# AIGeeksGroup/UniVid

Measured on AMD Instinct MI355X. Metric: denoise_steps_per_sec, higher is better.
Workload: dtype bf16

## Files before the change

### univid_amd/csrc/gemm_bf16_kernels.h

```cpp
#pragma once
#include "common.h"
#include <stdlib.h>
#include <type_traits>

const float* uv_zero_page();

#define UV_BK 64

enum {
    UV_EPI_BF16 = 0,
    UV_EPI_GELU_BF16 = 1,
    UV_EPI_F32_FROM_BF16 = 2,
    UV_EPI_RESID_F32 = 3,
    UV_EPI_GATE_RESID_F32 = 4,
    UV_EPI_BF16_T = 5,
    UV_EPI_BF16_SSQ = 6,
};

struct GemmArgs {
    const bf16_t* A;
    const bf16_t* W;
    const bf16_t* bias;
    void* out;
    const float* gate;
    const int32_t* gate_tid;
    const float* zeros;
    long lda, ldw, ldo, gate_stride;
    int M, N, K;
    int tiles_m, tiles_n;
    int gm;
    float* ssq;
    long ld_ssq;
    float* ws_slab;
    int* ws_cnt;
};

typedef __attribute__((address_space(3))) void lds_void;

__device__ __forceinline__ void glds16(const void* g, lds_void* l) {
    __builtin_amdgcn_global_load_lds(g, l, 16, 0, 0);
}

template <int EPI, bool F16 = false, bool FULL = false>
__device__ __forceinline__ void epi_frag(const GemmArgs& p, int mb, int nb, const f32x4& a, int frow, int fq) {
    if (EPI != UV_EPI_BF16_T) {
        const int m = mb + frow, n = nb + 4 * fq;
        if (!FULL && (m >= p.M || n >= p.N)) return;
        float v[4];
#pragma unroll
        for (int e = 0; e < 4; ++e) v[e] = a[e];
        if (FULL || p.bias) {
            const u32x2 bb = *(const u32x2*)((FULL && !p.bias) ? (const bf16_t*)p.zeros : p.bias + n);
            v[0] += in16<F16>((bf16_t)(bb[0] & 0xffff));
            v[1] += in16<F16>((bf16_t)(bb[0] >> 16));
            v[2] += in16<F16>((bf16_t)(bb[1] & 0xffff));
            v[3] += in16<F16>((bf16_t)(bb[1] >> 16));
        }
        if (EPI == UV_EPI_BF16) {
            u32x2 o = {pack16_2<F16>(v[0], v[1]), pack16_2<F16>(v[2], v[3])};
            *(u32x2*)((bf16_t*)p.out + (long)m * p.ldo + n) = o;
        } else if (EPI == UV_EPI_GELU_BF16) {
#pragma unroll
            for (int e = 0; e < 4; e += 2) {
                const uint32_t pk = pack16_2<F16>(v[e], v[e + 1]);
                const f32x2 y = gelu_tanh_f32x2((f32x2){in16<F16>((bf16_t)(pk & 0xffff)), in16<F16>((bf16_t)(pk >> 16))});
                v[e] = y[0];
                v[e + 1] = y[1];
            }
            u32x2 o = {pack16_2<F16>(v[0], v[1]), pack16_2<F16>(v[2], v[3])};
            *(u32x2*)((bf16_t*)p.out + (long)m * p.ldo + n) = o;
        } else if (EPI == UV_EPI_F32_FROM_BF16) {
            f32x4 o = {round16<F16>(v[0]), round16<F16>(v[1]), round16<F16>(v[2]), round16<F16>(v[3])};
            *(f32x4*)((float*)p.out + (long)m * p.ldo + n) = o;
        } else if (EPI == UV_EPI_RESID_F32) {
            float* xp = (float*)p.out + (long)m * p.ldo + n;
            f32x4 x = *(const f32x4*)xp;
#pragma unroll
            for (int e = 0; e < 4; ++e) x[e] = __fadd_rn(x[e], round16<F16>(v[e]));
            *(f32x4*)xp = x;
        } else if (EPI == UV_EPI_GATE_RESID_F32) {
            const int t = p.gate_tid ? p.gate_tid[m] : 0;
            const f32x4 g = *(const f32x4*)(p.gate + (long)t * p.gate_stride + n);
            float* xp = (float*)p.out + (long)m * p.ldo + n;
            f32x4 x = *(const f32x4*)xp;
#pragma unroll
            for (int e = 0; e < 4; ++e) x[e] = __fadd_rn(x[e], __fmul_rn(round16<F16>(v[e]), g[e]));
            *(f32x4*)xp = x;
        }
    } else {
        const int n = nb + frow, m = mb + 4 * fq;
        if (!FULL && (n >= p.N || m >= p.M)) return;
        const float b = FULL ? in16<F16>(*(p.bias ? p.bias + n : (const bf16_t*)p.zeros)) : (p.bias ? in16<F16>(p.bias[n]) : 0.f);
        bf16_t* op = (bf16_t*)p.out + (long)n * p.ldo + m;
        if (FULL || m + 3 < p.M) {
            u32x2 o = {pack16_2<F16>(a[0] + b, a[1] + b), pack16_2<F16>(a[2] + b, a[3] + b)};
            *(u32x2*)op = o;
        } else {
            for (int e = 0; e < 4 && m + e < p.M; ++e) op[e] = out16<F16>(a[e] + b);
        }
    }
}


__device__ __forceinline__ float ssq_group32(const float (&v0)[4], const float (&v1)[4]) {
    const float s0 = __fadd_rn(__fadd_rn(__fadd_rn(__fmul_rn(v0[0], v0[0]), __fmul_rn(v0[1], v0[1])), __fmul_rn(v0[2], v0[2])), __fmul_rn(v0[3], v0[3]));
    const float s1 = __fadd_rn(__fadd_rn(__fadd_rn(__fmul_rn(v1[0], v1[0]), __fmul_rn(v1[1], v1[1])), __fmul_rn(v1[2], v1[2])), __fmul_rn(v1[3], v1[3]));
    const float u = __fadd_rn(s0, s1);
    const float t = __fadd_rn(u, __shfl_xor(u, 16, 64));
    return __fadd_rn(t, __shfl_xor(t, 32, 64));
}

template <bool F16>
__device__ __forceinline__ void epi_pair_ssq(const GemmArgs& p, int mb, int nb, const f32x4& a0, const f32x4& a1, int frow, int fq) {
    const int m = mb + frow;
    float v[2][4];
#pragma unroll
    for (int f = 0; f < 2; ++f) {
        const int n = min(nb + 16 * f + 4 * fq, p.N - 4);
        const u32x2 bb = p.bias ? *(const u32x2*)(p.bias + n) : (u32x2){0u, 0u};
        const f32x4& a = f ? a1 : a0;
        v[f][0] = round16<F16>(a[0] + in16<F16>((bf16_t)(bb[0] & 0xffff)));
        v[f][1] = round16<F16>(a[1] + in16<F16>((bf16_t)(bb[0] >> 16)));
        v[f][2] = round16<F16>(a[2] + in16<F16>((bf16_t)(bb[1] & 0xffff)));
        v[f][3] = round16<F16>(a[3] + in16<F16>((bf16_t)(bb[1] >> 16)));
        if (m < p.M && nb + 16 * f + 4 * fq < p.N) {
            u32x2 o = {pack16_2<F16>(v[f][0], v[f][1]), pack16_2<F16>(v[f][2], v[f][3])};
            *(u32x2*)((bf16_t*)p.out + (long)m * p.ldo + nb + 16 * f + 4 * fq) = o;
        }
    }
    const float g = ssq_group32(v[0], v[1]);
    if (fq == 0 && m < p.M && nb < p.N) p.ssq[(long)m * p.ld_ssq + (nb >> 5)] = g;
}

template <int EPI, bool F16>
__device__ __forceinline__ void epi_pair16(const GemmArgs& p, int mb, int nb, const f32x4& a0, const f32x4& a1, int frow, int fq) {
    static_assert(EPI == UV_EPI_BF16 || EPI == UV_EPI_GELU_BF16 || EPI == UV_EPI_BF16_SSQ, "16-bit row-major outputs only");
    const int m = mb + frow;
    uint32_t w[2][2];
    float r[2][4];
#pragma unroll
    for (int f = 0; f < 2; ++f) {
        const int n = nb + 16 * f + 4 * fq;
        const u32x2 bb = *(const u32x2*)(p.bias ? p.bias + n : (const bf16_t*)p.zeros);
        const f32x4& a = f ? a1 : a0;
        float v[4] = {a[0] + in16<F16>((bf16_t)(bb[0] & 0xffff)), a[1] + in16<F16>((bf16_t)(bb[0] >> 16)),
                      a[2] + in16<F16>((bf16_t)(bb[1] & 0xffff)), a[3] + in16<F16>((bf16_t)(bb[1] >> 16))};
        if (EPI == UV_EPI_GELU_BF16) {
#pragma unroll
            for (int e = 0; e < 4; e += 2) {
                const uint32_t pk = pack16_2<F16>(v[e], v[e + 1]);
                const f32x2 r = {in16<F16>((bf16_t)(pk & 0xffff)), in16<F16>((bf16_t)(pk >> 16))};
                const f32x2 y = gelu_tanh_f32x2(r);
                v[e] = y[0];
                v[e + 1] = y[1];
            }
        }
        if (EPI == UV_EPI_BF16_SSQ) {
#pragma unroll
            for (int e = 0; e < 4; ++e) r[f][e] = v[e] = round16<F16>(v[e]);
        }
        w[f][0] = pack16_2<F16>(v[0], v[1]);
        w[f][1] = pack16_2<F16>(v[2], v[3]);
    }
    if (EPI == UV_EPI_BF16_SSQ) {
        const float g = ssq_group32(r[0], r[1]);
        if (fq == 0) p.ssq[(long)m * p.ld_ssq + (nb >> 5)] = g;
    }
    const auto s0 = __builtin_amdgcn_permlane16_swap(w[0][0], w[1][0], false, false);
    const auto s1 = __builtin_amdgcn_permlane16_swap(w[0][1], w[1][1], false, false);
    const u32x4 o = {(uint32_t)s0[0], (uint32_t)s1[0], (uint32_t)s0[1], (uint32_t)s1[1]};
    const int col = ((fq & 1) << 4) + ((fq >> 1) << 3);
    *(u32x4*)((bf16_t*)p.out + (long)m * p.ldo + nb + col) = o;
}

template <bool F16>
__device__ __forceinline__ void epi_pair16_T(const GemmArgs& p, int mb, int nb, const f32x4& a0, const f32x4& a1, int frow, int fq) {
    const int n = nb + frow;
    const float b = in16<F16>(*(p.bias ? p.bias + n : (const bf16_t*)p.zeros));
    uint32_t w0[2] = {pack16_2<F16>(a0[0] + b, a0[1] + b), pack16_2<F16>(a0[2] + b, a0[3] + b)};
    uint32_t w1[2] = {pack16_2<F16>(a1[0] + b, a1[1] + b), pack16_2<F16>(a1[2] + b, a1[3] + b)};
    const auto s0 = __builtin_amdgcn_permlane16_swap(w0[0], w1[0], false, false);
    const auto s1 = __builtin_amdgcn_permlane16_swap(w0[1], w1[1], false, false);
    const u32x4 o = {(uint32_t)s0[0], (uint32_t)s1[0], (uint32_t)s0[1], (uint32_t)s1[1]};
    const int row = ((fq & 1) << 4) + ((fq >> 1) << 3);
    *(u32x4*)((bf16_t*)p.out + (long)n * p.ldo + mb + row) = o;
}

template <int EPI, int NF, int D, bool F16 = false>
__device__ __forceinline__ void epi_rmw_pipe(const GemmArgs& p, const int (&mb)[NF], const int (&nb)[NF], const f32x4 (&acc)[NF],
                                             int frow, int fq) {
    static_assert(EPI == UV_EPI_RESID_F32 || EPI == UV_EPI_GATE_RESID_F32, "rmw epilogues only");
    constexpr bool GATE = EPI == UV_EPI_GATE_RESID_F32;
    const float* grow[NF];
    if (GATE) {
        int t[NF];
#pragma unroll
        for (int f = 0; f < NF; ++f) t[f] = p.gate_tid ? p.gate_tid[min(mb[f] + frow, p.M - 1)] : 0;
#pragma unroll
        for (int f = 0; f < NF; ++f) grow[f] = p.gate + (long)t[f] * p.gate_stride;
    }
    f32x4 xb[D], gb[D];
    u32x2 bb[D];
    auto issue = [&](int f, int slot) {
        const int m = min(mb[f] + frow, p.M - 1), n = min(nb[f] + 4 * fq, p.N - 4);
        xb[slot] = *(const f32x4*)((const float*)p.out + (long)m * p.ldo + n);
        if (GATE) gb[slot] = *(const f32x4*)(grow[f] + n);
        bb[slot] = p.bias ? *(const u32x2*)(p.bias + n) : (u32x2){0u, 0u};
    };
#pragma unroll
    for (int f = 0; f < D && f < NF; ++f) issue(f, f);
#pragma unroll
    for (int f = 0; f < NF; ++f) {
        const int slot = f % D;
        const int m = mb[f] + frow, n = nb[f] + 4 * fq;
        float v[4];
        v[0] = acc[f][0] + in16<F16>((bf16_t)(bb[slot][0] & 0xffff));
        v[1] = acc[f][1] + in16<F16>((bf16_t)(bb[slot][0] >> 16));
        v[2] = acc[f][2] + in16<F16>((bf16_t)(bb[slot][1] & 0xffff));
        v[3] = acc[f][3] + in16<F16>((bf16_t)(bb[slot][1] >> 16));
        f32x4 x = xb[slot];
#pragma unroll
        for (int e = 0; e < 4; ++e)
            x[e] = GATE ? __fadd_rn(x[e], __fmul_rn(round16<F16>(v[e]), gb[slot][e])) : __fadd_rn(x[e], round16<F16>(v[e]));
        if (m < p.M && n < p.N) *(f32x4*)((float*)p.out + (long)m * p.ldo + n) = x;
        if (f + D < NF) issue(f + D, slot);
    }
}

template <int BM, int BN, int WM, int WN, int EPI, int NS = 2, bool F16 = false>
__global__ __launch_bounds__(WM* WN * 64) void gemm_bf16_nt_kernel(GemmArgs p) {
    constexpr int NW = WM * WN;
    constexpr int NT = NW * 64;
    constexpr int TM = BM / WM / 16;
    constexpr int TN = BN / WN / 16;
    constexpr int A_BYTES = BM * 128;
    constexpr int W_BYTES = BN * 128;
    constexpr int STAGE_BYTES = A_BYTES + W_BYTES;
    constexpr int A_INSTR = (BM / 8 + NW - 1) / NW;
    constexpr int W_INSTR = (BN / 8 + NW - 1) / NW;
    static_assert(BM % 8 == 0 && BN % 8 == 0 && (BM / WM) % 16 == 0 && (BN / WN) % 16 == 0, "tile/wave mismatch");
    constexpr bool TRANS = (EPI == UV_EPI_BF16_T);

    extern __shared__ __attribute__((aligned(16))) char smem[];

    const int tid = threadIdx.x;
    const int lane = tid & 63;
    const int wave = __builtin_amdgcn_readfirstlane(tid >> 6);
    const int wm = wave / WN, wn = wave % WN;

    const int nblk = p.tiles_m * p.tiles_n;
    int bid = blockIdx.x;
    {
        const int q = nblk >> 3, r = nblk & 7, xcd = bid & 7, idx = bid >> 3;
        bid = (xcd < r ? xcd * (q + 1) : r * (q + 1) + (xcd - r) * q) + idx;
    }
    constexpr int GM = 4;
    const int group_sz = GM * p.tiles_n;
    const int group = bid / group_sz;
    const int first_m = group * GM;
    const int gm = min(GM, p.tiles_m - first_m);
    const int in_group = bid - group * group_sz;
    const int tile_m = first_m + in_group % gm;
    const int tile_n = in_group / gm;
    const int m0 = tile_m * BM, n0 = tile_n * BN;

    const int srow = lane >> 3;
    const int pchunk = lane & 7;
    const bf16_t* a_src[A_INSTR];
    const bf16_t* w_src[W_INSTR];
#pragma unroll
    for (int i = 0; i < A_INSTR; ++i) {
        const int row = (i * NW + wave) * 8 + srow;
        const int c = pchunk ^ ((row >> 1) & 7);
        const int gr = min(m0 + row, p.M - 1);
        a_src[i] = p.A + (long)gr * p.lda + c * 8;
    }
#pragma unroll
    for (int i = 0; i < W_INSTR; ++i) {
        const int row = (i * NW + wave) * 8 + srow;
        const int c = pchunk ^ ((row >> 1) & 7);
        const int gr = min(n0 + row, p.N - 1);
        w_src[i] = p.W + (long)gr * p.ldw + c * 8;
    }

    auto stage = [&](int kt, int buf) {
        char* base = smem + buf * STAGE_BYTES;
        const int koff = kt * UV_BK;
#pragma unroll
        for (int i = 0; i < A_INSTR; ++i)
            if ((i * NW + wave) * 8 < BM) glds16(a_src[i] + koff, (lds_void*)(base + (i * NW + wave) * 1024));
#pragma unroll
        for (int i = 0; i < W_INSTR; ++i)
            if ((i * NW + wave) * 8 < BN) glds16(w_src[i] + koff, (lds_void*)(base + A_BYTES + (i * NW + wave) * 1024));
    };

    f32x4 acc[TN][TM];
#pragma unroll
    for (int i = 0; i < TN; ++i)
#pragma unroll
        for (int j = 0; j < TM; ++j) acc[i][j] = (f32x4){0.f, 0.f, 0.f, 0.f};

    const int frow = lane & 15;
    const int fq = lane >> 4;
    int a_off[TM], w_off[TN];
    int a_key[TM], w_key[TN];
#pragma unroll
    for (int j = 0; j < TM; ++j) {
        const int row = wm * (BM / WM) + j * 16 + frow;
        a_off[j] = row * 128;
        a_key[j] = (row >> 1) & 7;
    }
#pragma unroll
    for (int i = 0; i < TN; ++i) {
        const int row = wn * (BN / WN) + i * 16 + frow;
        w_off[i] = A_BYTES + row * 128;
        w_key[i] = (row >> 1) & 7;
    }

    const int nk = p.K / UV_BK;
    auto compute = [&](const char* base) {
#pragma unroll
        for (int ks = 0; ks < 2; ++ks) {
            bf16x8 af[TM], wf[TN];
            const int c = ks * 4 + fq;
#pragma unroll
            for (int j = 0; j < TM; ++j)
                af[j] = *(const bf16x8*)(base + a_off[j] + ((c ^ a_key[j]) << 4));
#pragma unroll
            for (int i = 0; i < TN; ++i)
                wf[i] = *(const bf16x8*)(base + w_off[i] + ((c ^ w_key[i]) << 4));
#pragma unroll
            for (int i = 0; i < TN; ++i)
#pragma unroll
                for (int j = 0; j < TM; ++j) {
                    if (TRANS)
                        acc[i][j] = mfma_16x16x32<F16>(af[j], wf[i], acc[i][j]);
                    else
                        acc[i][j] = mfma_16x16x32<F16>(wf[i], af[j], acc[i][j]);
                }
        }
    };
    if constexpr (NS == 2) {
        stage(0, 0);
        asm volatile("s_waitcnt vmcnt(0)" ::: "memory");
        __syncthreads();
        for (int kt = 0; kt < nk; ++kt) {
            const int buf = kt & 1;
            if (kt + 1 < nk) stage(kt + 1, buf ^ 1);
            compute(smem + buf * STAGE_BYTES);
            asm volatile("s_waitcnt vmcnt(0)" ::: "memory");
            __syncthreads();
        }
    } else {
        static_assert(BM % (8 * NW) == 0 && BN % (8 * NW) == 0, "ring variant needs unguarded staging");
        constexpr int LPS = A_INSTR + W_INSTR;
        static_assert((NS - 2) * LPS < 64, "vmcnt range");
#pragma unroll
        for (int s0 = 0; s0 < NS - 1; ++s0)
            if (s0 < nk) stage(s0, s0);
        int buf = 0, nbuf = NS - 1;
        for (int kt = 0; kt < nk; ++kt) {
            if (kt + NS - 2 < nk) {
                asm volatile("s_waitcnt vmcnt(%0)" ::"n"((NS - 2) * LPS) : "memory");
            } else {
                asm volatile("s_waitcnt vmcnt(0)" ::: "memory");
            }
            __builtin_amdgcn_s_barrier();
            if (kt + NS - 1 < nk) stage(kt + NS - 1, nbuf);
            compute(smem + buf * STAGE_BYTES);
            buf = buf + 1 == NS ? 0 : buf + 1;
            nbuf = nbuf + 1 == NS ? 0 : nbuf + 1;
        }
    }

    if constexpr (EPI == UV_EPI_RESID_F32 || EPI == UV_EPI_GATE_RESID_F32) {
        constexpr int NF = TM * TN;
        int mb[NF], nb[NF];
        f32x4 av[NF];
#pragma unroll
        for (int j = 0; j < TM; ++j)
#pragma unroll
            for (int i = 0; i < TN; ++i) {
                mb[j * TN + i] = m0 + wm * (BM / WM) + j * 16;
                nb[j * TN + i] = n0 + wn * (BN / WN) + i * 16;
                av[j * TN + i] = acc[i][j];
            }
        epi_rmw_pipe<EPI, NF, (NF >= 8 ? 4 : 2), F16>(p, mb, nb, av, frow, fq);
    } else if constexpr (EPI == UV_EPI_BF16_SSQ) {
        static_assert(TN % 2 == 0 && (BN / WN) % 32 == 0, "UV_EPI_BF16_SSQ needs whole 32-column groups per wave");
#pragma unroll
        for (int j = 0; j < TM; ++j)
#pragma unroll
            for (int i = 0; i < TN; i += 2)
                epi_pair_ssq<F16>(p, m0 + wm * (BM / WM) + j * 16, n0 + wn * (BN / WN) + i * 16, acc[i][j], acc[i + 1][j], frow, fq);
    } else {
#pragma unroll
        for (int j = 0; j < TM; ++j)
#pragma unroll
            for (int i = 0; i < TN; ++i)
                epi_frag<EPI, F16>(p, m0 + wm * (BM / WM) + j * 16, n0 + wn * (BN / WN) + i * 16, acc[i][j], frow, fq);
    }
}


template <int EPI, bool F16>
__device__ __forceinline__ void epi_rmw_rows_lds(const GemmArgs& p, char* smem, const f32x4 (&acc)[2][2][2][4], int m0, int n0,
                                                 int wave, int lane) {
    static_assert(EPI == UV_EPI_RESID_F32 || EPI == UV_EPI_GATE_RESID_F32, "rmw epilogues only");
    constexpr bool GATE = EPI == UV_EPI_GATE_RESID_F32;
    constexpr int D = 8;
    const int wr = wave >> 2, wc = wave & 3;
    const int frow = lane & 15, fq = lane >> 4;
    float bv[2][2][4];
#pragma unroll
    for (int hn = 0; hn < 2; ++hn)
#pragma unroll
        for (int i = 0; i < 2; ++i) {
            const int n = min(n0 + hn * 128 + wc * 32 + i * 16 + 4 * fq, p.N - 4);
            const u32x2 bb = p.bias ? *(const u32x2*)(p.bias + n) : (u32x2){0u, 0u};
            bv[hn][i][0] = in16<F16>((bf16_t)(bb[0] & 0xffff));
            bv[hn][i][1] = in16<F16>((bf16_t)(bb[0] >> 16));
            bv[hn][i][2] = in16<F16>((bf16_t)(bb[1] & 0xffff));
            bv[hn][i][3] = in16<F16>((bf16_t)(bb[1] >> 16));
        }
    const int n = n0 + 4 * lane;
    const bool n_ok = n < p.N;
    const int nc = min(n, p.N - 4);
#pragma unroll
    for (int h = 0; h < 2; ++h) {
#pragma unroll
        for (int j = 0; j < 4; ++j)
#pragma unroll
            for (int hn = 0; hn < 2; ++hn)
#pragma unroll
                for (int i = 0; i < 2; ++i) {
                    const int row = wr * 64 + j * 16 + frow;
                    const int chunk = hn * 32 + wc * 8 + i * 4 + fq;
                    f32x4 y;
#pragma unroll
                    for (int e = 0; e < 4; ++e) y[e] = round16<F16>(acc[hn][h][i][j][e] + bv[hn][i][e]);
                    *(f32x4*)(smem + row * 1024 + ((chunk ^ (row & 7)) << 4)) = y;
                }
        asm volatile("s_waitcnt lgkmcnt(0)" ::: "memory");
        __builtin_amdgcn_s_barrier();
        const int mbase = m0 + h * 128 + wave * 16;
        f32x4 xb[D], gb[D];
        int tid16 = 0;
        if (GATE && p.gate_tid) tid16 = p.gate_tid[min(mbase + (lane & 15), p.M - 1)];
        auto issue = [&](int rr, int slot) {
            const int m = min(mbase + rr, p.M - 1);
            xb[slot] = *(const f32x4*)((const float*)p.out + (long)m * p.ldo + nc);
            if (GATE) {
                const int t = __builtin_amdgcn_readlane(tid16, rr);
                gb[slot] = *(const f32x4*)(p.gate + (long)t * p.gate_stride + nc);
            }
        };
#pragma unroll
        for (int rr = 0; rr < D; ++rr) issue(rr, rr);
#pragma unroll
        for (int rr = 0; rr < 16; ++rr) {
            const int slot = rr % D;
            const int row = wave * 16 + rr;
            const f32x4 y = *(const f32x4*)(smem + row * 1024 + ((lane ^ (row & 7)) << 4));
            f32x4 x = xb[slot];
#pragma unroll
            for (int e = 0; e < 4; ++e) x[e] = GATE ? __fadd_rn(x[e], __fmul_rn(y[e], gb[slot][e])) : __fadd_rn(x[e], y[e]);
            if (mbase + rr < p.M && n_ok) *(f32x4*)((float*)p.out + (long)(mbase + rr) * p.ldo + n) = x;
            if (rr + D < 16) issue(rr + D, slot);
        }
        if (h == 0) {
            asm volatile("s_waitcnt lgkmcnt(0)" ::: "memory");
            __builtin_amdgcn_s_barrier();
        }
    }
}

#define UV_SB() __builtin_amdgcn_s_barrier()
#define UV_SCHED() __builtin_amdgcn_sched_barrier(0)

template <int EPI, int VAR = 0, bool F16 = false, int SK = 1>
__global__ __launch_bounds__(512) void gemm_bf16_8ph_kernel(GemmArgs p) {
    static_assert(SK == 1 || (VAR == 5 && (8 % SK) == 0), "split-K: VAR 5, SK in {2, 4, 8}");
    constexpr bool TRANS = (EPI == UV_EPI_BF16_T);
    constexpr int HALF = 16384;
    constexpr int BUF = 4 * HALF;
    extern __shared__ __attribute__((aligned(16))) char smem[];

    const int tid = threadIdx.x;
    const int lane = tid & 63;
    const int wave = __builtin_amdgcn_readfirstlane(tid >> 6);
    const int wr = wave >> 2, wc = wave & 3;

    const int nblk = p.tiles_m * p.tiles_n;
    int bid = blockIdx.x;
    int slice = 0;
    if constexpr (SK == 1) {
        const int q = nblk >> 3, r = nblk & 7, xcd = bid & 7, idx = bid >> 3;
        bid = (xcd < r ? xcd * (q + 1) : r * (q + 1) + (xcd - r) * q) + idx;
    } else {
        const int xcd = bid & 7, idx = bid >> 3, per = gridDim.x >> 3;
        const int u = xcd * per + idx;
        slice = u % SK;
        bid = u / SK;
        if (bid >= nblk) return;
    }
    constexpr int GM = 4;
    const int group_sz = GM * p.tiles_n;
    const int group = bid / group_sz;
    const int first_m = group * GM;
    const int gm = min(GM, p.tiles_m - first_m);
    const int in_group = bid - group * group_sz;
    const int m0 = (first_m + in_group % gm) * 256, n0 = (in_group / gm) * 256;
    const int kbeg = SK == 1 ? 0 : slice * (p.K / SK);

    const int srow = lane >> 3, pchunk = lane & 7;
    const bf16_t* a_src[2][2];
    const bf16_t* w_src[2][2];
#pragma unroll
    for (int h = 0; h < 2; ++h)
#pragma unroll
        for (int i = 0; i < 2; ++i) {
            const int row = (i * 8 + wave) * 8 + srow;
            const int c = pchunk ^ ((row >> 1) & 7);
            a_src[h][i] = p.A + (long)min(m0 + h * 128 + row, p.M - 1) * p.lda + c * 8 + kbeg;
            w_src[h][i] = p.W + (long)min(n0 + h * 128 + row, p.N - 1) * p.ldw + c * 8 + kbeg;
        }
    char* const my_dst = smem + wave * 1024;
    const int nk = p.K / SK / UV_BK;
#define UV_STAGE(SRC, KT, DSTOFF)                                         \
    {                                                                     \
        const bf16_t* g0_ = SRC[0] + (long)(KT) * UV_BK;                  \
        const bf16_t* g1_ = SRC[1] + (long)(KT) * UV_BK;                  \
        glds16(g0_, (lds_void*)(my_dst + (DSTOFF)));                      \
        glds16(g1_, (lds_void*)(my_dst + (DSTOFF) + 8192));              \
    }

    const int frow = lane & 15, fq = lane >> 4;
    const int lx = (fq ^ (frow >> 1)) << 4;
    const char* const la = smem + (wr * 64 + frow) * 128;
    const char* const lw = smem + 2 * HALF + (wc * 32 + frow) * 128;

    f32x4 acc[2][2][2][4];
#pragma unroll
    for (int a = 0; a < 2; ++a)
#pragma unroll
        for (int b = 0; b < 2; ++b)
#pragma unroll
            for (int i = 0; i < 2; ++i)
#pragma unroll
                for (int j = 0; j < 4; ++j) acc[a][b][i][j] = (f32x4){0.f, 0.f, 0.f, 0.f};
    bf16x8 af[4][2], w0[2][2], w1[2][2];

#define UV_RD_A(B, H)                                                                             \
    _Pragma("unroll") for (int j = 0; j < 4; ++j) {                                                                     \
        af[j][0] = *(const bf16x8*)(la + (B) * BUF + (H) * HALF + j * 2048 + lx);                 \
        af[j][1] = *(const bf16x8*)(la + (B) * BUF + (H) * HALF + j * 2048 + (lx ^ 64));          \
    }
#define UV_RD_W(B, H, WF)                                                                         \
    _Pragma("unroll") for (int i = 0; i < 2; ++i) {                                                                     \
        WF[i][0] = *(const bf16x8*)(lw + (B) * BUF + (H) * HALF + i * 2048 + lx);                 \
        WF[i][1] = *(const bf16x8*)(lw + (B) * BUF + (H) * HALF + i * 2048 + (lx ^ 64));          \
    }
#define UV_MFMA_H(HM, HN, WF, KS)                                                                 \
    _Pragma("unroll") for (int i = 0; i < 2; ++i)                                                 \
    _Pragma("unroll") for (int j = 0; j < 4; ++j) {                                               \
        if (TRANS)                                                                                \
            acc[HN][HM][i][j] = mfma_16x16x32<F16>(af[j][KS], WF[i][KS], acc[HN][HM][i][j]); \
        else                                                                                      \
            acc[HN][HM][i][j] = mfma_16x16x32<F16>(WF[i][KS], af[j][KS], acc[HN][HM][i][j]); \
    }
#define UV_MFMA_Q(HM, HN, WF)                                                                     \
    __builtin_amdgcn_s_setprio(1);                                                                \
    UV_MFMA_H(HM, HN, WF, 0) UV_MFMA_H(HM, HN, WF, 1)                                             \
    __builtin_amdgcn_s_setprio(0);
#define UV_LGKM0() asm volatile("s_waitcnt lgkmcnt(0)" ::: "memory")
#define UV_KTILE0(T, B, O, ST1, ST2)                                                              \
    UV_RD_W(B, 0, w0) UV_SCHED(); UV_RD_A(B, 0)                                                   \
    if (ST1) UV_STAGE(a_src[1], (T) + 1, (O) * BUF + HALF)                                        \
    asm volatile("s_waitcnt lgkmcnt(8)" ::: "memory");                                            \
    UV_SB(); UV_LGKM0(); UV_SCHED();                                                              \
    UV_MFMA_Q(0, 0, w0) UV_SCHED(); UV_SB();                                                      \
    UV_RD_W(B, 1, w1)                                                                             \
    if (ST2) UV_STAGE(w_src[0], (T) + 2, (B) * BUF + 2 * HALF)                                    \
    UV_SB(); UV_LGKM0(); UV_SCHED();                                                              \
    UV_MFMA_Q(0, 1, w1) UV_SCHED(); UV_SB();                                                      \
    UV_RD_A(B, 1)                                                                                 \
    if (ST2) UV_STAGE(a_src[0], (T) + 2, (B) * BUF)                                               \
    UV_SB(); UV_LGKM0(); UV_SCHED();                                                              \
    UV_MFMA_Q(1, 1, w1) UV_SCHED(); UV_SB();                                                      \
    if (ST2) {                                                                                    \
        UV_STAGE(w_src[1], (T) + 2, (B) * BUF + 3 * HALF)                                         \
        asm volatile("s_waitcnt vmcnt(6)" ::: "memory");                                          \
    } else {                                                                                      \
        asm volatile("s_waitcnt vmcnt(0)" ::: "memory");                                          \
    }                                                                                             \
    UV_SB(); UV_SCHED();                                                                          \
    UV_MFMA_Q(1, 0, w0) UV_SCHED(); UV_SB();
#define UV_KTILE5(T, B, O, ST1, ST2) UV_KTILE5X((T) + 1, (T) + 2, B, O, ST1, ST2)
#define UV_KTILE5X(K1, K2, B, O, ST1, ST2)                                                        \
    UV_RD_W(B, 0, w0) UV_RD_W(B, 1, w1) UV_RD_A(B, 0)                                             \
    if (ST1) {                                                                                    \
        UV_STAGE(w_src[0], K1, (O) * BUF + 2 * HALF)                                              \
        UV_STAGE(a_src[1], K1, (O) * BUF + HALF)                                                  \
        asm volatile("s_waitcnt vmcnt(8)" ::: "memory");                                          \
    } else {                                                                                      \
        asm volatile("s_waitcnt vmcnt(0)" ::: "memory");                                          \
    }                                                                                             \
    UV_LGKM0(); UV_SB(); UV_SCHED();                                                              \
    __builtin_amdgcn_s_setprio(1);                                                                \
    UV_MFMA_H(0, 0, w0, 0) UV_MFMA_H(0, 0, w0, 1) UV_MFMA_H(0, 1, w1, 0) UV_MFMA_H(0, 1, w1, 1)   \
    __builtin_amdgcn_s_setprio(0); UV_SCHED(); UV_SB();                                           \
    UV_RD_A(B, 1)                                                                                 \
    if (ST2) {                                                                                    \
        UV_STAGE(w_src[1], K2, (B) * BUF + 3 * HALF)                                              \
        UV_STAGE(a_src[0], K2, (B) * BUF)                                                         \
        asm volatile("s_waitcnt vmcnt(6)" ::: "memory");                                          \
    } else if (ST1) {                                                                             \
        asm volatile("s_waitcnt vmcnt(2)" ::: "memory");                                          \
    } else {                                                                                      \
        asm volatile("s_waitcnt vmcnt(0)" ::: "memory");                                          \
    }                                                                                             \
    UV_LGKM0(); UV_SB(); UV_SCHED();                                                              \
    __builtin_amdgcn_s_setprio(1);                                                                \
    UV_MFMA_H(1, 1, w1, 0) UV_MFMA_H(1, 1, w1, 1) UV_MFMA_H(1, 0, w0, 0) UV_MFMA_H(1, 0, w0, 1)   \
    __builtin_amdgcn_s_setprio(0); UV_SCHED(); UV_SB();
#define UV_KTILE(T, B, O, ST1, ST2)                                                               \
    if constexpr (VAR == 5) { UV_KTILE5(T, B, O, ST1, ST2) } else { UV_KTILE0(T, B, O, ST1, ST2) }

    if constexpr (VAR == 5) {
        UV_STAGE(w_src[0], 0, 2 * HALF) UV_STAGE(w_src[1], 0, 3 * HALF) UV_STAGE(a_src[0], 0, 0) UV_STAGE(a_src[1], 0, HALF)
        UV_STAGE(w_src[1], 1, BUF + 3 * HALF) UV_STAGE(a_src[0], 1, BUF)
        asm volatile("s_waitcnt vmcnt(6)" ::: "memory");
    } else {
        UV_STAGE(w_src[0], 0, 2 * HALF) UV_STAGE(a_src[0], 0, 0) UV_STAGE(w_src[1], 0, 3 * HALF) UV_STAGE(a_src[1], 0, HALF)
        UV_STAGE(w_src[0], 1, BUF + 2 * HALF) UV_STAGE(a_src[0], 1, BUF) UV_STAGE(w_src[1], 1, BUF + 3 * HALF)
        asm volatile("s_waitcnt vmcnt(6)" ::: "memory");
    }
    UV_SB();
    if (wr == 1) UV_SB();

    int t = 0;
    for (; t + 2 < nk; t += 2) {
        UV_KTILE(t, 0, 1, true, true)
        UV_KTILE(t + 1, 1, 0, true, true)
    }
    UV_KTILE(t, 0, 1, true, false)
    UV_KTILE(t + 1, 1, 0, false, false)
    if (wr == 0) UV_SB();

    if constexpr (SK > 1) {
        f32x4* const accf = &acc[0][0][0][0];
        const auto slabs = __builtin_amdgcn_make_buffer_rsrc(p.ws_slab + (long)bid * SK * 65536, 0, SK * 262144, 0x00020000);
        const int voff = tid * 16;
        const int row_lim = p.M - m0 - wr * 64;
#pragma unroll
        for (int f = 0; f < 32; ++f)
            if (((f >> 3) & 1) * 128 + (f & 3) * 16 < row_lim)
                __builtin_amdgcn_raw_buffer_store_b128(__builtin_bit_cast(u32x4, accf[f]), slabs, voff, slice * 262144 + f * 8192, 0);
        asm volatile("s_waitcnt vmcnt(0) lgkmcnt(0)" ::: "memory");
        __builtin_amdgcn_s_barrier();
        if (tid == 0) {
            __builtin_amdgcn_fence(__ATOMIC_RELEASE, "agent");
            asm volatile("s_waitcnt vmcnt(0)" ::: "memory");
            const int ticket = __hip_atomic_fetch_add(p.ws_cnt + bid, 1, __ATOMIC_RELAXED, __HIP_MEMORY_SCOPE_AGENT);
            if (ticket == SK - 1) {
                __builtin_amdgcn_fence(__ATOMIC_ACQUIRE, "agent");
                asm volatile("s_waitcnt vmcnt(0)" ::: "memory");
            }
            *(volatile int*)smem = ticket;
        }
        asm volatile("s_waitcnt lgkmcnt(0)" ::: "memory");
        __builtin_amdgcn_s_barrier();
        const int ticket = __builtin_amdgcn_readfirstlane(*(volatile int*)smem);
        if (ticket != SK - 1) return;
        asm volatile("s_waitcnt lgkmcnt(0)" ::: "memory");
        __builtin_amdgcn_s_barrier();
        constexpr int G = 4;
#pragma unroll
        for (int f0 = 0; f0 < 32; f0 += G) {
            f32x4 v[G][SK];
#pragma unroll
            for (int g = 0; g < G; ++g)
#pragma unroll
                for (int sl = 0; sl < SK; ++sl) {
                    v[g][sl] = (f32x4){0.f, 0.f, 0.f, 0.f};
                    if ((((f0 + g) >> 3) & 1) * 128 + ((f0 + g) & 3) * 16 < row_lim)
                        v[g][sl] = __builtin_bit_cast(f32x4, __builtin_amdgcn_raw_buffer_load_b128(slabs, voff, sl * 262144 + (f0 + g) * 8192, 0));
                }
#pragma unroll
            for (int g = 0; g < G; ++g) {
                f32x4 sum = v[g][0];
#pragma unroll
                for (int sl = 1; sl < SK; ++sl)
#pragma unroll
                    for (int e = 0; e < 4; ++e) sum[e] = __fadd_rn(sum[e], v[g][sl][e]);
                asm volatile("" : "+v"(sum));
                accf[f0 + g] = sum;
            }
            asm volatile("" ::: "memory");
            __builtin_amdgcn_sched_barrier(0);
        }
    }

    if constexpr ((EPI == UV_EPI_RESID_F32 || EPI == UV_EPI_GATE_RESID_F32) && VAR != 0) {
        asm volatile("s_waitcnt lgkmcnt(0)" ::: "memory");
        __builtin_amdgcn_s_barrier();
        epi_rmw_rows_lds<EPI, F16>(p, smem, acc, m0, n0, wave, lane);
    } else if constexpr (EPI == UV_EPI_RESID_F32 || EPI == UV_EPI_GATE_RESID_F32) {
        int mb[32], nb[32];
        f32x4 av[32];
#pragma unroll
        for (int hm = 0; hm < 2; ++hm)
#pragma unroll
            for (int j = 0; j < 4; ++j)
#pragma unroll
                for (int hn = 0; hn < 2; ++hn)
#pragma unroll
                    for (int i = 0; i < 2; ++i) {
                        const int f = ((hm * 4 + j) * 2 + hn) * 2 + i;
                        mb[f] = m0 + hm * 128 + wr * 64 + j * 16;
                        nb[f] = n0 + hn * 128 + wc * 32 + i * 16;
                        av[f] = acc[hn][hm][i][j];
                    }
        epi_rmw_pipe<EPI, 32, 8, F16>(p, mb, nb, av, frow, fq);
    } else if constexpr (EPI == UV_EPI_BF16_SSQ) {
#pragma unroll
        for (int hm = 0; hm < 2; ++hm)
#pragma unroll
            for (int j = 0; j < 4; ++j)
#pragma unroll
                for (int hn = 0; hn < 2; ++hn)
                    epi_pair_ssq<F16>(p, m0 + hm * 128 + wr * 64 + j * 16, n0 + hn * 128 + wc * 32, acc[hn][hm][0][j], acc[hn][hm][1][j], frow, fq);
    } else {
#pragma unroll
        for (int hm = 0; hm < 2; ++hm)
#pragma unroll
            for (int j = 0; j < 4; ++j)
#pragma unroll
                for (int hn = 0; hn < 2; ++hn)
#pragma unroll
                    for (int i = 0; i < 2; ++i)
                        epi_frag<EPI, F16>(p, m0 + hm * 128 + wr * 64 + j * 16, n0 + hn * 128 + wc * 32 + i * 16, acc[hn][hm][i][j], frow, fq);
    }
}

template <int EPI, bool F16 = false>
__global__ __launch_bounds__(512) void gemm_bf16_8ph_persist_kernel(GemmArgs p) {
    constexpr bool TRANS = (EPI == UV_EPI_BF16_T);
    constexpr bool RMW = (EPI == UV_EPI_RESID_F32 || EPI == UV_EPI_GATE_RESID_F32);
    constexpr int VAR = 5;
    constexpr int HALF = 16384;
    constexpr int BUF = 4 * HALF;
    extern __shared__ __attribute__((aligned(16))) char smem[];

    const int tid = threadIdx.x;
    const int lane = tid & 63;
    const int wave = __builtin_amdgcn_readfirstlane(tid >> 6);
    const int wr = wave >> 2, wc = wave & 3;

    const int nblk = p.tiles_m * p.tiles_n;
    const int G = gridDim.x >> 3;
    int first, cnt;
    {
        const int q = nblk >> 3, r = nblk & 7, xcd = blockIdx.x & 7;
        first = xcd < r ? xcd * (q + 1) : r * (q + 1) + (xcd - r) * q;
        cnt = q + (xcd < r ? 1 : 0);
    }
    int cur = blockIdx.x >> 3;
    if (cur >= cnt) return;
    const int GM = p.gm;
    const int group_sz = GM * p.tiles_n;
    auto origin = [&](int bid, int& m0, int& n0) {
        const int group = bid / group_sz;
        const int first_m = group * GM;
        const int gm = min(GM, p.tiles_m - first_m);
        const int in_group = bid - group * group_sz;
        m0 = (first_m + in_group % gm) * 256;
        n0 = (in_group / gm) * 256;
    };
    int m0, n0;
    origin(first + cur, m0, n0);

    const int srow = lane >> 3, pchunk = lane & 7;
    const bf16_t* a_src[2][2];
    const bf16_t* w_src[2][2];
#pragma unroll
    for (int h = 0; h < 2; ++h)
#pragma unroll
        for (int i = 0; i < 2; ++i) {
            const int row = (i * 8 + wave) * 8 + srow;
            const int c = pchunk ^ ((row >> 1) & 7);
            a_src[h][i] = p.A + (long)(m0 + h * 128 + row) * p.lda + c * 8;
            w_src[h][i] = p.W + (long)(n0 + h * 128 + row) * p.ldw + c * 8;
        }
    char* const my_dst = smem + wave * 1024;
    const int nk = p.K / UV_BK;
    const int frow = lane & 15, fq = lane >> 4;
    const int lx = (fq ^ (frow >> 1)) << 4;
    const char* const la = smem + (wr * 64 + frow) * 128;
    const char* const lw = smem + 2 * HALF + (wc * 32 + frow) * 128;
    f32x4 acc[2][2][2][4];
    bf16x8 af[4][2], w0[2][2], w1[2][2];

    auto move_ptrs = [&](const bf16_t* (&src)[2], long d) { src[0] += d; src[1] += d; };
    bool fresh = true;
    for (;;) {
        if (fresh) {
            UV_STAGE(w_src[0], 0, 2 * HALF) UV_STAGE(w_src[1], 0, 3 * HALF) UV_STAGE(a_src[0], 0, 0) UV_STAGE(a_src[1], 0, HALF)
            UV_STAGE(w_src[1], 1, BUF + 3 * HALF) UV_STAGE(a_src[0], 1, BUF)
            asm volatile("s_waitcnt vmcnt(6)" ::: "memory");
            UV_SB();
        }
        fresh = RMW;
        if (wr == 1) UV_SB();
#pragma unroll
        for (int a = 0; a < 2; ++a)
#pragma unroll
            for (int b = 0; b < 2; ++b)
#pragma unroll
                for (int i = 0; i < 2; ++i)
#pragma unroll
                    for (int j = 0; j < 4; ++j) acc[a][b][i][j] = (f32x4){0.f, 0.f, 0.f, 0.f};

        const int nxt = cur + G;
        const bool has_next = nxt < cnt;
        int m1 = m0, n1 = n0;
        long dA = 0, dW = 0;
        if (has_next) {
            origin(first + nxt, m1, n1);
            dA = (long)(m1 - m0) * p.lda;
            dW = (long)(n1 - n0) * p.ldw;
        }
        int t = 0;
        for (; t + 2 < nk; t += 2) {
            UV_KTILE5(t, 0, 1, true, true)
            UV_KTILE5(t + 1, 1, 0, true, true)
        }
        if constexpr (!RMW) {
            move_ptrs(w_src[1], dW); move_ptrs(a_src[0], dA);
            UV_KTILE5X(nk - 1, 0, 0, 1, true, true)
            move_ptrs(w_src[0], dW);
            move_ptrs(a_src[1], dA);
            UV_KTILE5X(0, 1, 1, 0, true, true)
        } else {
            UV_KTILE5(t, 0, 1, true, false)
            UV_KTILE5(t + 1, 1, 0, false, false)
            move_ptrs(w_src[0], dW); move_ptrs(w_src[1], dW); move_ptrs(a_src[0], dA); move_ptrs(a_src[1], dA);
        }
        if (wr == 0) UV_SB();

        if constexpr (RMW) {
            asm volatile("s_waitcnt lgkmcnt(0)" ::: "memory");
            __builtin_amdgcn_s_barrier();
            epi_rmw_rows_lds<EPI, F16>(p, smem, acc, m0, n0, wave, lane);
            if (has_next) {
                asm volatile("s_waitcnt lgkmcnt(0)" ::: "memory");
                __builtin_amdgcn_s_barrier();
            }
        } else if constexpr (EPI == UV_EPI_BF16 || EPI == UV_EPI_GELU_BF16 || EPI == UV_EPI_BF16_SSQ) {
#pragma unroll
            for (int hm = 0; hm < 2; ++hm)
#pragma unroll
                for (int j = 0; j < 4; ++j)
#pragma unroll
                    for (int hn = 0; hn < 2; ++hn)
                        epi_pair16<EPI, F16>(p, m0 + hm * 128 + wr * 64 + j * 16, n0 + hn * 128 + wc * 32, acc[hn][hm][0][j], acc[hn][hm][1][j], frow, fq);
        } else if constexpr (EPI == UV_EPI_BF16_T) {
#pragma unroll
            for (int hm = 0; hm < 2; ++hm)
#pragma unroll
                for (int j = 0; j < 4; j += 2)
#pragma unroll
                    for (int hn = 0; hn < 2; ++hn)
#pragma unroll
                        for (int i = 0; i < 2; ++i)
                            epi_pair16_T<F16>(p, m0 + hm * 128 + wr * 64 + j * 16, n0 + hn * 128 + wc * 32 + i * 16, acc[hn][hm][i][j], acc[hn][hm][i][j + 1], frow, fq);
        } else {
#pragma unroll
            for (int hm = 0; hm < 2; ++hm)
#pragma unroll
                for (int j = 0; j < 4; ++j)
#pragma unroll
                    for (int hn = 0; hn < 2; ++hn)
#pragma unroll
                        for (int i = 0; i < 2; ++i)
                            epi_frag<EPI, F16, true>(p, m0 + hm * 128 + wr * 64 + j * 16, n0 + hn * 128 + wc * 32 + i * 16, acc[hn][hm][i][j], frow, fq);
        }
        if (!has_next) break;
        m0 = m1; n0 = n1; cur = nxt;
    }
    asm volatile("s_waitcnt vmcnt(0)" ::: "memory");
}


template <void (*KERN)(GemmArgs)>
static int launch_kernel(dim3 grid, dim3 block, size_t lds, hipStream_t stream, const GemmArgs& a, const char* who) {
    UV_ONCE_PER_DEVICE(hipFuncSetAttribute((const void*)KERN, hipFuncAttributeMaxDynamicSharedMemorySize, (int)lds));
    hipLaunchKernelGGL(KERN, grid, block, lds, stream, a);
    UV_CHECK_LAUNCH(who);
    return 0;
}

constexpr unsigned UV_EPIS_ALL = 0x7f;
constexpr bool epi_in(unsigned epis, int e) { return e >= 0 && e < 32 && (epis >> e & 1) != 0; }
template <int E>
using epi_c = std::integral_constant<int, E>;
template <unsigned EPIS = UV_EPIS_ALL, class Launch>
static int launch_epi(int epi, Launch&& launch) {
    switch (epi) {
        case UV_EPI_BF16: if constexpr (epi_in(EPIS, UV_EPI_BF16)) return launch(epi_c<UV_EPI_BF16>()); break;
        case UV_EPI_GELU_BF16: if constexpr (epi_in(EPIS, UV_EPI_GELU_BF16)) return launch(epi_c<UV_EPI_GELU_BF16>()); break;
        case UV_EPI_F32_FROM_BF16: if constexpr (epi_in(EPIS, UV_EPI_F32_FROM_BF16)) return launch(epi_c<UV_EPI_F32_FROM_BF16>()); break;
        case UV_EPI_RESID_F32: if constexpr (epi_in(EPIS, UV_EPI_RESID_F32)) return launch(epi_c<UV_EPI_RESID_F32>()); break;
        case UV_EPI_GATE_RESID_F32: if constexpr (epi_in(EPIS, UV_EPI_GATE_RESID_F32)) return launch(epi_c<UV_EPI_GATE_RESID_F32>()); break;
        case UV_EPI_BF16_T: if constexpr (epi_in(EPIS, UV_EPI_BF16_T)) return launch(epi_c<UV_EPI_BF16_T>()); break;
        case UV_EPI_BF16_SSQ: if constexpr (epi_in(EPIS, UV_EPI_BF16_SSQ)) return launch(epi_c<UV_EPI_BF16_SSQ>()); break;
    }
    uv_set_error("uv_gemm_bf16_nt: unknown epilogue %d", epi);
    return -1;
}

template <int VAR = 0, bool F16 = false>
static int launch_8ph(const GemmArgs& a0, int epi, hipStream_t stream) {
    GemmArgs a = a0;
    a.tiles_m = (a.M + 255) / 256;
    a.tiles_n = (a.N + 255) / 256;
    const dim3 grid(a.tiles_m * a.tiles_n);
    return launch_epi(epi, [&](auto e) {
        return launch_kernel<gemm_bf16_8ph_kernel<decltype(e)::value, VAR, F16>>(grid, 512, 128 * 1024, stream, a, "uv_gemm_bf16_nt");
    });
}

static inline long splitk_ws_bytes(int M, int N, int sk) { return 4096 + (long)((M + 255) / 256) * ((N + 255) / 256) * sk * 262144L; }

template <int SK, bool F16 = false>
static int launch_8ph_splitk(const GemmArgs& a0, int epi, hipStream_t stream, void* ws, long ws_bytes) {
    GemmArgs a = a0;
    a.tiles_m = (a.M + 255) / 256;
    a.tiles_n = (a.N + 255) / 256;
    const int tiles = a.tiles_m * a.tiles_n;
    UV_CHECK_ARG(a.K % (SK * 128) == 0 && a.K / SK >= 256, "uv_gemm_bf16_nt_ws: split-K %d needs K %% %d == 0 and K / %d >= 256 (K=%d)", SK, SK * 128, SK, a.K);
    UV_CHECK_ARG(tiles <= 1024, "uv_gemm_bf16_nt_ws: split-K serves leftover strips (at most 1024 tiles; %d here)", tiles);
    UV_CHECK_ARG(ws && ((uintptr_t)ws & 255) == 0 && ws_bytes >= splitk_ws_bytes(a.M, a.N, SK),
                 "uv_gemm_bf16_nt_ws: workspace of %ld bytes (256-byte aligned) needed, %ld given", splitk_ws_bytes(a.M, a.N, SK), ws_bytes);
    constexpr unsigned EPIS = 1u << UV_EPI_BF16 | 1u << UV_EPI_RESID_F32 | 1u << UV_EPI_GATE_RESID_F32;
    UV_CHECK_ARG(epi_in(EPIS, epi),
                 "uv_gemm_bf16_nt_ws: the split-K strip is built for the bf16 and the residual epilogues (0, 3, 4), not %d", epi);
    a.ws_cnt = (int*)ws;
    a.ws_slab = (float*)((char*)ws + 4096);
    if (hipMemsetAsync(a.ws_cnt, 0, (size_t)tiles * sizeof(int), stream) != hipSuccess) {
        uv_set_error("uv_gemm_bf16_nt_ws: hipMemsetAsync of the tile counters failed");
        return -1;
    }
    const dim3 grid(8 * ((tiles * SK + 7) / 8));
    return launch_epi<EPIS>(epi, [&](auto e) {
        return launch_kernel<gemm_bf16_8ph_kernel<decltype(e)::value, 5, F16, SK>>(grid, 512, 128 * 1024, stream, a, "uv_gemm_bf16_nt_ws");
    });
}

template <bool F16 = false>
static int launch_8ph_persist(const GemmArgs& a0, int epi, hipStream_t stream) {
    GemmArgs a = a0;
    UV_CHECK_ARG(a.M % 256 == 0 && a.N % 256 == 0, "uv_gemm_bf16_nt: the persistent kernel needs whole 256x256 tiles (M=%d N=%d)", a.M, a.N);
    UV_CHECK_ARG(a.ldo % 8 == 0 || (epi != UV_EPI_BF16_T && epi != UV_EPI_BF16 && epi != UV_EPI_GELU_BF16 && epi != UV_EPI_BF16_SSQ),
                 "uv_gemm_bf16_nt: the persistent kernel stores 16 bytes per lane: ldo=%ld must be a multiple of 8 elements", a.ldo);
    a.tiles_m = a.M / 256;
    a.tiles_n = a.N / 256;
    a.gm = (a.N <= 4096 && a.K <= 4096) ? 8 : (a.K >= 8192 ? 2 : 4);
    if (const int gm = uv_option(UV_OPT_GEMM_GM); gm > 0) a.gm = gm;
    const int tiles = a.tiles_m * a.tiles_n;
    int wgs = uv_num_cus() & ~7;
    if (wgs > tiles) wgs = tiles & ~7;
    UV_CHECK_ARG(wgs >= 8, "uv_gemm_bf16_nt: too few tiles (%d) for the persistent kernel", tiles);
    const dim3 grid(wgs);
    return launch_epi(epi, [&](auto e) {
        return launch_kernel<gemm_bf16_8ph_persist_kernel<decltype(e)::value, F16>>(grid, 512, 128 * 1024, stream, a, "uv_gemm_bf16_nt");
    });
}

template <int BM, int BN, int WM, int WN, int NS = 2, bool F16 = false>
static int launch_cfg(const GemmArgs& a0, int epi, hipStream_t stream) {
    GemmArgs a = a0;
    a.tiles_m = (a.M + BM - 1) / BM;
    a.tiles_n = (a.N + BN - 1) / BN;
    constexpr bool SSQ = (BN / WN) % 32 == 0;
    UV_CHECK_ARG(SSQ || epi != UV_EPI_BF16_SSQ, "uv_gemm_bf16_nt_ssq: this tile shape has no whole 32-column groups per wave");
    const dim3 grid(a.tiles_m * a.tiles_n);
    return launch_epi<SSQ ? UV_EPIS_ALL : UV_EPIS_ALL & ~(1u << UV_EPI_BF16_SSQ)>(epi, [&](auto e) {
        return launch_kernel<gemm_bf16_nt_kernel<BM, BN, WM, WN, decltype(e)::value, NS, F16>>(grid, WM * WN * 64, NS * (BM + BN) * 128, stream, a, "uv_gemm_bf16_nt");
    });
}
```

Before: 3.960.

## Restructure residual RMW epilogue: overlap residual loads with LDS staging, defer bias

The residual/gated-residual epilogue now issues all 16 residual row loads interleaved with writing accumulator fragments to LDS, instead of loading them after the barrier with a depth-8 ring. The bias add and bf16 rounding move from the per-fragment staging side to the per-row output side, so one bias vector per lane is loaded instead of four. A separate path handles a per-column gate with no token index, loading it once. This is meant to hide global load latency behind LDS stores and cut bias loads, at the cost of more registers held live (16 f32x4 residual buffers).

```diff
diff --git a/univid_amd/csrc/gemm_bf16_kernels.h b/univid_amd/csrc/gemm_bf16_kernels.h
--- a/univid_amd/csrc/gemm_bf16_kernels.h
+++ b/univid_amd/csrc/gemm_bf16_kernels.h
@@ -405,68 +405,84 @@
 
 template <int EPI, bool F16>
 __device__ __forceinline__ void epi_rmw_rows_lds(const GemmArgs& p, char* smem, const f32x4 (&acc)[2][2][2][4], int m0, int n0,
-                                                 int wave, int lane) {
+                                                 int wave) {
     static_assert(EPI == UV_EPI_RESID_F32 || EPI == UV_EPI_GATE_RESID_F32, "rmw epilogues only");
     constexpr bool GATE = EPI == UV_EPI_GATE_RESID_F32;
-    constexpr int D = 8;
+    constexpr int R = 16;
+    constexpr int DG = 8;
+    int lane;
+    asm volatile("v_mbcnt_lo_u32_b32 %0, -1, 0\n\tv_mbcnt_hi_u32_b32 %0, -1, %0" : "=v"(lane));
     const int wr = wave >> 2, wc = wave & 3;
     const int frow = lane & 15, fq = lane >> 4;
-    float bv[2][2][4];
-#pragma unroll
-    for (int hn = 0; hn < 2; ++hn)
-#pragma unroll
-        for (int i = 0; i < 2; ++i) {
-            const int n = min(n0 + hn * 128 + wc * 32 + i * 16 + 4 * fq, p.N - 4);
-            const u32x2 bb = p.bias ? *(const u32x2*)(p.bias + n) : (u32x2){0u, 0u};
-            bv[hn][i][0] = in16<F16>((bf16_t)(bb[0] & 0xffff));
-            bv[hn][i][1] = in16<F16>((bf16_t)(bb[0] >> 16));
-            bv[hn][i][2] = in16<F16>((bf16_t)(bb[1] & 0xffff));
-            bv[hn][i][3] = in16<F16>((bf16_t)(bb[1] >> 16));
-        }
     const int n = n0 + 4 * lane;
     const bool n_ok = n < p.N;
     const int nc = min(n, p.N - 4);
+    const bool row_gate = GATE && p.gate_tid != nullptr;
+    u32x2 bb = {0u, 0u};
+    f32x4 g0 = {1.f, 1.f, 1.f, 1.f};
 #pragma unroll
     for (int h = 0; h < 2; ++h) {
-#pragma unroll
-        for (int j = 0; j < 4; ++j)
+        const int mbase = m0 + h * 128 + wave * 16;
+        f32x4 xb[R];
+        auto load_x = [&](int rr) { xb[rr] = *(const f32x4*)((const float*)p.out + (long)min(mbase + rr, p.M - 1) * p.ldo + nc); };
+        auto stage_y = [&](int j) {
 #pragma unroll
             for (int hn = 0; hn < 2; ++hn)
 #pragma unroll
                 for (int i = 0; i < 2; ++i) {
                     const int row = wr * 64 + j * 16 + frow;
                     const int chunk = hn * 32 + wc * 8 + i * 4 + fq;
-                    f32x4 y;
-#pragma unroll
-                    for (int e = 0; e < 4; ++e) y[e] = round16<F16>(acc[hn][h][i][j][e] + bv[hn][i][e]);
-                    *(f32x4*)(smem + row * 1024 + ((chunk ^ (row & 7)) << 4)) = y;
+                    *(f32x4*)(smem + row * 1024 + ((chunk ^ (row & 7)) << 4)) = acc[hn][h][i][j];
                 }
+        };
+        stage_y(0);
+        __builtin_amdgcn_sched_barrier(0);
+        if (h == 0) {
+            if (p.bias) bb = *(const u32x2*)(p.bias + nc);
+            if (GATE && !row_gate) g0 = *(const f32x4*)(p.gate + nc);
+        }
+        int tid16 = 0;
+        if (row_gate) tid16 = p.gate_tid[min(mbase + (lane & 15), p.M - 1)];
+#pragma unroll
+        for (int j = 1; j < 4; ++j) {
+#pragma unroll
+            for (int rr = 4 * (j - 1); rr < (j == 3 ? R : 4 * j); ++rr) load_x(rr);
+            __builtin_amdgcn_sched_barrier(0);
+            stage_y(j);
+        }
         asm volatile("s_waitcnt lgkmcnt(0)" ::: "memory");
         __builtin_amdgcn_s_barrier();
-        const int mbase = m0 + h * 128 + wave * 16;
-        f32x4 xb[D], gb[D];
-        int tid16 = 0;
-        if (GATE && p.gate_tid) tid16 = p.gate_tid[min(mbase + (lane & 15), p.M - 1)];
-        auto issue = [&](int rr, int slot) {
-            const int m = min(mbase + rr, p.M - 1);
-            xb[slot] = *(const f32x4*)((const float*)p.out + (long)m * p.ldo + nc);
-            if (GATE) {
+        __builtin_amdgcn_sched_barrier(0);
+        const float bv[4] = {in16<F16>((bf16_t)(bb[0] & 0xffff)), in16<F16>((bf16_t)(bb[0] >> 16)), in16<F16>((bf16_t)(bb[1] & 0xffff)),
+                             in16<F16>((bf16_t)(bb[1] >> 16))};
+        auto row_out = [&](int rr, const f32x4& g) {
+            const int row = wave * 16 + rr;
+            const f32x4 a = *(const f32x4*)(smem + row * 1024 + ((lane ^ (row & 7)) << 4));
+            f32x4 x = xb[rr];
+#pragma unroll
+            for (int e = 0; e < 4; ++e) {
+                const float y = round16<F16>(a[e] + bv[e]);
+                x[e] = GATE ? __fadd_rn(x[e], __fmul_rn(y, g[e])) : __fadd_rn(x[e], y);
+            }
+            if (mbase + rr < p.M && n_ok) *(f32x4*)((float*)p.out + (long)(mbase + rr) * p.ldo + n) = x;
+        };
+        if (row_gate) {
+            f32x4 gb[DG];
+            auto issue = [&](int rr) {
                 const int t = __builtin_amdgcn_readlane(tid16, rr);
-                gb[slot] = *(const f32x4*)(p.gate + (long)t * p.gate_stride + nc);
+                gb[rr % DG] = *(const f32x4*)(p.gate + (long)t * p.gate_stride + nc);
+            };
+#pragma unroll
+            for (int rr = 0; rr < DG; ++rr) issue(rr);
+#pragma unroll
+            for (int rr = 0; rr < R; ++rr) {
+                row_out(rr, gb[rr % DG]);
+                if (rr + DG < R) issue(rr + DG);
             }
-        };
-#pragma unroll
-        for (int rr = 0; rr < D; ++rr) issue(rr, rr);
-#pragma unroll
-        for (int rr = 0; rr < 16; ++rr) {
-            const int slot = rr % D;
-            const int row = wave * 16 + rr;
-            const f32x4 y = *(const f32x4*)(smem + row * 1024 + ((lane ^ (row & 7)) << 4));
-            f32x4 x = xb[slot];
-#pragma unroll
-            for (int e = 0; e < 4; ++e) x[e] = GATE ? __fadd_rn(x[e], __fmul_rn(y[e], gb[slot][e])) : __fadd_rn(x[e], y[e]);
-            if (mbase + rr < p.M && n_ok) *(f32x4*)((float*)p.out + (long)(mbase + rr) * p.ldo + n) = x;
-            if (rr + D < 16) issue(rr + D, slot);
+        } else {
+#pragma unroll
+            for (int rr = 0; rr < R; ++rr) row_out(rr, g0);
+            asm volatile("" ::: "memory");
         }
         if (h == 0) {
             asm volatile("s_waitcnt lgkmcnt(0)" ::: "memory");
@@ -705,7 +721,7 @@
     if constexpr ((EPI == UV_EPI_RESID_F32 || EPI == UV_EPI_GATE_RESID_F32) && VAR != 0) {
         asm volatile("s_waitcnt lgkmcnt(0)" ::: "memory");
         __builtin_amdgcn_s_barrier();
-        epi_rmw_rows_lds<EPI, F16>(p, smem, acc, m0, n0, wave, lane);
+        epi_rmw_rows_lds<EPI, F16>(p, smem, acc, m0, n0, wave);
     } else if constexpr (EPI == UV_EPI_RESID_F32 || EPI == UV_EPI_GATE_RESID_F32) {
         int mb[32], nb[32];
         f32x4 av[32];
@@ -852,7 +868,7 @@
         if constexpr (RMW) {
             asm volatile("s_waitcnt lgkmcnt(0)" ::: "memory");
             __builtin_amdgcn_s_barrier();
-            epi_rmw_rows_lds<EPI, F16>(p, smem, acc, m0, n0, wave, lane);
+            epi_rmw_rows_lds<EPI, F16>(p, smem, acc, m0, n0, wave);
             if (has_next) {
                 asm volatile("s_waitcnt lgkmcnt(0)" ::: "memory");
                 __builtin_amdgcn_s_barrier();
```

Measured after the change: 3.965 (median of 6 runs). No clear change (+0.1%).
